# astojanov/Clover

Hardware: AMD Instinct MI355X
Metric: int4 GEMV (CloverMatrix4::mvm) effective GB/s, algorithmic operand bytes / time (higher is better)
Workload: dtype int4; 1 GPU; CloverMatrix4::mvm 65536x65536 int4 (65536x65536 per GPU; preset c3: BASELINE configs[2] per GPU), x and result CloverVector4, STOCHASTIC_ROUNDING_DISABLED, bit-exact reference order; rows_per_gpu=65536, cols=65536, parallelism=row-shard x1, settle_launches=168

## Files before the change

### clover_amd/csrc/matrix4.hip

```cpp
#include "rng_device.h"

#include <stdlib.h>
#include <string.h>


#define MVM_CHUNK 65536u

template <int U, bool NT>
__device__ __forceinline__ void mvm_steps(const u32x4 *__restrict__ Ap, const u32x4 *xs, const float *cs, int q,
                                          uint32_t t0, float &a0, float &a1, float &a2, float &a3)
{
    u32x4 a[U];
#pragma unroll
    for (int u = 0; u < U; u++) a[u] = NT ? __builtin_nontemporal_load(&Ap[4 * (t0 + u) + q]) : Ap[4 * (t0 + u) + q];
#pragma unroll
    for (int u = 0; u < U; u++) {
        const u32x4 xv = xs[4 * (t0 + u) + q];
        const float c = cs[2 * (t0 + u) + (q >> 1)];
        a0 = __builtin_fmaf(c, (float)sdot8(a[u].x, xv.x, 0), a0);
        a1 = __builtin_fmaf(c, (float)sdot8(a[u].y, xv.y, 0), a1);
        a2 = __builtin_fmaf(c, (float)sdot8(a[u].z, xv.z, 0), a2);
        a3 = __builtin_fmaf(c, (float)sdot8(a[u].w, xv.w, 0), a3);
    }
}

template <int U, bool NT>
__device__ __forceinline__ void mvm_steps8(const u32x2 *__restrict__ Ap, const u32x2 *xs, const float *cs, int e, uint32_t t0, float &a0,
                                           float &a1)
{
    u32x2 a[U];
#pragma unroll
    for (int u = 0; u < U; u++) a[u] = NT ? __builtin_nontemporal_load(&Ap[8 * (t0 + u) + e]) : Ap[8 * (t0 + u) + e];
#pragma unroll
    for (int u = 0; u < U; u++) {
        const u32x2 xv = xs[8 * (t0 + u) + e];
        const float c = cs[2 * (t0 + u) + (e >> 2)];
        a0 = __builtin_fmaf(c, (float)sdot8(a[u].x, xv.x, 0), a0);
        a1 = __builtin_fmaf(c, (float)sdot8(a[u].y, xv.y, 0), a1);
    }
}

__device__ __forceinline__ int requantize_wave(float d, float noise, uint32_t *r_words, float *sr, float *scale)
{
    const int lane = threadIdx.x & 63;
    float m = wave_max(__builtin_fabsf(d));
    m = fix_zero_max(m);
    const float k = 7.0f / m;
    const int qv = quant1(d, k, noise);
    if (r_words) {
        uint32_t w = ((uint32_t)qv & 0xFu) << nib_shift(lane & 7);
        w |= __shfl_xor(w, 1);
        w |= __shfl_xor(w, 2);
        w |= __shfl_xor(w, 4);
        if ((lane & 7) == 0) r_words[lane >> 3] = w;
        if (lane == 0) *sr = m;
    }
    *scale = m;
    return qv;
}

struct MvmFuse {
    const uint32_t *qu;
    const float *su;
    float a;
    uint32_t *r2;
    float *sr2;
};

template <int U, bool NT, bool ST, bool FUSE, int L = 4>
__global__ __launch_bounds__(64 * L) void k_m4_mvm64(const uint8_t *__restrict__ A, const float *__restrict__ sA,
                                                  uint64_t cols, const uint8_t *__restrict__ x, const float *__restrict__ sx,
                                                  float *__restrict__ d_out, uint32_t *r, float *sr,
                                                  uint64_t *rng_state, uint64_t seq, const uint64_t *__restrict__ pow_rows, MvmFuse fuse)
{
    extern __shared__ __attribute__((aligned(16))) char smem[];
    u32x4 *xs = reinterpret_cast<u32x4 *>(smem);
    float *cs = reinterpret_cast<float *>(smem + MVM_CHUNK / 2);
    float *dsh = cs + MVM_CHUNK / 64;
    uint64_t *rbase = reinterpret_cast<uint64_t *>(dsh + 64);
    uint64_t *raw = rbase + 4;
    uint64_t *rbase2 = raw + 8, *raw2 = rbase2 + 4;
    if (ST) {
        const uint64_t a0 = rng_workgroup_begin(rng_state, seq, pow_rows, blockIdx.x, 1, (FUSE ? 4ull : 2ull) * gridDim.x, rbase);
        if (FUSE) {
            const uint64_t b2 = wave_pow_apply(pow_rows, a0, (uint64_t)gridDim.x + blockIdx.x, 1);
            if ((threadIdx.x & 63) == 0) rbase2[threadIdx.x >> 6] = b2;
        }
    }
    uint32_t fuse_w = 0;
    float fuse_s = 0.0f;
    if (FUSE && threadIdx.x < 64) {
        fuse_w = fuse.qu[blockIdx.x * 8 + (threadIdx.x >> 3)];
        fuse_s = fuse.su[blockIdx.x];
    }

    static_assert(L == 4 || (L == 8 && !ST), "the stochastic epilogue assumes 4 waves");
    constexpr int THREADS = 64 * L;
    const uint64_t rb = blockIdx.x;
    const int tid = threadIdx.x;
    const int q = tid & (L - 1);
    const int rho = tid / L;
    const uint64_t row = rb * 64 + rho;
    const u32x4 *Arow = reinterpret_cast<const u32x4 *>(A + row * (cols / 2));
    const float *sArow = sA + rb * (cols / 64);

    float a0 = 0.0f, a1 = 0.0f, a2 = 0.0f, a3 = 0.0f;

    for (uint64_t c0 = 0; c0 < cols; c0 += MVM_CHUNK) {
        const uint32_t cw = (uint32_t)((cols - c0) < MVM_CHUNK ? (cols - c0) : MVM_CHUNK);
        if (c0) __syncthreads();
        const u32x4 *xg = reinterpret_cast<const u32x4 *>(x + c0 / 2);
        {
            constexpr int NX = MVM_CHUNK / 32 / THREADS;
            constexpr int NC = MVM_CHUNK / 64 / THREADS;
            u32x4 xr[NX];
            float sa[NC], sv[NC];
            const uint32_t nx = cw / 32, nc = cw / 64;
#pragma unroll
            for (int k = 0; k < NX; k++) { const uint32_t i = tid + THREADS * k; xr[k] = xg[i < nx ? i : 0]; }
#pragma unroll
            for (int k = 0; k < NC; k++) {
                const uint32_t i = tid + THREADS * k, ii = i < nc ? i : 0;
                sa[k] = sArow[c0 / 64 + ii];
                sv[k] = sx[c0 / 64 + ii];
            }
#pragma unroll
            for (int k = 0; k < NX; k++) { const uint32_t i = tid + THREADS * k; if (i < nx) xs[i] = xr[k]; }
#pragma unroll
            for (int k = 0; k < NC; k++) { const uint32_t i = tid + THREADS * k; if (i < nc) cs[i] = (sa[k] * CLV_RCP49) * sv[k]; }
        }
        __syncthreads();

        const u32x4 *Ap = Arow + c0 / 32;
        const uint32_t npairs = cw / 128;
        uint32_t t = 0;
        if constexpr (L == 4) {
            for (; t + U <= npairs; t += U) mvm_steps<U, NT>(Ap, xs, cs, q, t, a0, a1, a2, a3);
            for (; t < npairs; t++) mvm_steps<1, NT>(Ap, xs, cs, q, t, a0, a1, a2, a3);
        } else {
            const u32x2 *Ap8 = reinterpret_cast<const u32x2 *>(Ap);
            const u32x2 *xs8 = reinterpret_cast<const u32x2 *>(xs);
            for (; t + U <= npairs; t += U) mvm_steps8<U, NT>(Ap8, xs8, cs, q, t, a0, a1);
            for (; t < npairs; t++) mvm_steps8<1, NT>(Ap8, xs8, cs, q, t, a0, a1);
        }
    }

    const float v0 = a0 + __shfl_xor(a0, 2);
    const float v1 = a1 + __shfl_xor(a1, 2);
    const float v2 = a2 + __shfl_xor(a2, 2);
    const float v3 = a3 + __shfl_xor(a3, 2);
    const float x0 = v0 + __shfl_xor(v0, 1);
    const float x1 = v1 + __shfl_xor(v1, 1);
    const float x2 = v2 + __shfl_xor(v2, 1);
    const float x3 = v3 + __shfl_xor(v3, 1);
    float dot = (x0 + x2) + (x1 + x3);
    if constexpr (L == 8) {
        const float u0 = a0 + __shfl_xor(a0, 4), u1 = a1 + __shfl_xor(a1, 4);
        const float y0 = u0 + __shfl_xor(u0, 2), y1 = u1 + __shfl_xor(u1, 2);
        const float z0 = y0 + __shfl_xor(y0, 1), z1 = y1 + __shfl_xor(y1, 1);
        dot = z0 + z1;
    }

    if (q == 0) {
        dsh[rho] = dot;
        if (d_out) d_out[row] = dot;
    }
    if (ST && tid < 4) {
        gen_blocks(rbase[tid], 1, raw, tid);
        if (FUSE) gen_blocks(rbase2[tid], 1, raw2, tid);
    }
    __syncthreads();
    if ((r || FUSE) && tid < 64) {
        float noise = 0.0f;
        if (ST) {
            const int grp = tid & 7, j = tid >> 3;
            noise = noise_of(reinterpret_cast<const uint32_t *>(raw + (size_t)(grp >> 2) * 4)[j], grp & 3);
        }
        float m;
        const int qv = requantize_wave(dsh[tid], noise, r ? r + rb * 8 : nullptr, r ? sr + rb : nullptr, &m);
        if (FUSE) {
            const float su7 = div7(fuse_s), sv7 = div7(m * fuse.a);
            const float val = __builtin_fmaf((float)qv, sv7, (float)unpack1(fuse_w, tid & 7) * su7);
            float noise2 = 0.0f;
            if (ST) {
                const int g = (tid & 7) ^ 1, j = tid >> 3;
                noise2 = noise_of(reinterpret_cast<const uint32_t *>(raw2 + (size_t)(g >> 2) * 4)[j], g & 3);
            }
            float m2;
            requantize_wave(val, noise2, fuse.r2 + rb * 8, fuse.sr2 + rb, &m2);
        }
    }
}

__global__ __launch_bounds__(256) void k_m4_quantize_strip(const float *__restrict__ A, uint64_t cols, uint32_t *__restrict__ q,
                                                           float *__restrict__ s, uint32_t strips_x, uint32_t tiles_x)
{
    __shared__ float sh[4][4];
    const uint32_t sj = blockIdx.x % strips_x;
    const uint64_t bi = blockIdx.x / strips_x;
    const int wave = threadIdx.x >> 6, lane = threadIdx.x & 63;
    const uint64_t col = (uint64_t)sj * 256 + 4 * lane;
    const bool live = col < cols;
    const uint64_t row0 = bi * 64 + wave * 16;

    f32x4 v[16];
    float m = 0.0f;
#pragma unroll
    for (int r = 0; r < 16; r++) {
        v[r] = live ? __builtin_nontemporal_load(reinterpret_cast<const f32x4 *>(A + (row0 + r) * cols + col)) : f32x4{0.0f, 0.0f, 0.0f, 0.0f};
        m = fmaxf(m, fmaxf(fmaxf(__builtin_fabsf(v[r].x), __builtin_fabsf(v[r].y)), fmaxf(__builtin_fabsf(v[r].z), __builtin_fabsf(v[r].w))));
    }
    m = row16_max(m);
    if ((lane & 15) == 0) sh[wave][lane >> 4] = m;
    __syncthreads();
    const int t = lane >> 4;
    m = fix_zero_max(fmaxf(fmaxf(sh[0][t], sh[1][t]), fmaxf(sh[2][t], sh[3][t])));
    const float k = 7.0f / m;
    if (wave == 0 && (lane & 15) == 0 && live) s[bi * tiles_x + sj * 4 + t] = m;
    const int odd = lane & 1;
#pragma unroll
    for (int r = 0; r < 16; r += 2) {
        const uint32_t h0 = quant_pack4(v[r], k), h1 = quant_pack4(v[r + 1], k);
        const uint32_t give = odd ? h0 : h1;
        const uint32_t recv = (uint32_t)__builtin_amdgcn_update_dpp(0, (int)give, 0xB1, 0xF, 0xF, false);
        const uint32_t word = odd ? (recv | (h1 << 16)) : (h0 | (recv << 16));
        if (live) __builtin_nontemporal_store(word, &q[((row0 + r + odd) * cols + (col & ~7ull)) / 8]);
    }
}

__global__ __launch_bounds__(256) void k_m4_gemm_simple(const uint8_t *__restrict__ A, const float *__restrict__ sA, uint64_t M,
                                                        uint64_t K, const uint8_t *__restrict__ B, const float *__restrict__ sB,
                                                        uint64_t N, float *__restrict__ C)
{
    const uint64_t j = (uint64_t)blockIdx.x * 16 + (threadIdx.x & 15);
    const uint64_t i = (uint64_t)blockIdx.y * 16 + (threadIdx.x >> 4);
    if (i >= M || j >= N) return;
    const uint64_t kb = K / 64;
    const u32x4 *a = reinterpret_cast<const u32x4 *>(A + i * (K / 2));
    const u32x4 *b = reinterpret_cast<const u32x4 *>(B + j * (K / 2));
    const float *sa = sA + (i >> 6) * kb;
    const float *sb = sB + (j >> 6) * kb;
    float acc = 0.0f;
    for (uint64_t blk = 0; blk < kb; blk++) {
        const int S = dot32(a[2 * blk], b[2 * blk]) + dot32(a[2 * blk + 1], b[2 * blk + 1]);
        const float c = (sa[blk] * CLV_RCP49) * sb[blk];
        acc = __builtin_fmaf(c, (float)S, acc);
    }
    C[i * N + j] = acc;
}

template <bool NT>
__global__ __launch_bounds__(256) void k_m4_restore(const uint32_t *__restrict__ q, const float *__restrict__ s, f32x4 *__restrict__ A,
                                                    uint64_t nquads, uint64_t cols)
{
    const uint64_t f0 = ((uint64_t)blockIdx.x * 4 + (threadIdx.x >> 6)) * 256;
    const int lane = threadIdx.x & 63;
    const uint64_t tiles_x = cols / 64;
    uint32_t wd[4];
    float sc[4];
#pragma unroll
    for (int j = 0; j < 4; j++) {
        const uint64_t f = f0 + 64 * j + lane, fc = f < nquads ? f : 0;
        const uint64_t e = fc * 4, row = e / cols, col = e - row * cols;
        wd[j] = q[fc >> 1];
        sc[j] = s[(row >> 6) * tiles_x + (col >> 6)];
    }
#pragma unroll
    for (int j = 0; j < 4; j++) {
        const uint64_t f = f0 + 64 * j + lane;
        const uint32_t hw = wd[j] >> (16 * (lane & 1));
        const float k = div7(sc[j]);
        f32x4 v;
        v.x = (float)(((int)(hw << 24)) >> 28) * k;
        v.y = (float)(((int)(hw << 28)) >> 28) * k;
        v.z = (float)(((int)(hw << 16)) >> 28) * k;
        v.w = (float)(((int)(hw << 20)) >> 28) * k;
        if (f < nquads) {
            if (NT) __builtin_nontemporal_store(v, &A[f]);
            else A[f] = v;
        }
    }
}

int clm4_quantize_stochastic(const float *A, uint64_t rows, uint64_t cols, int8_t *q, float *s, uint64_t *rng, hipStream_t st);
int clm4_gemm_mfma(const int8_t *A, const float *sA, uint64_t M, uint64_t K, const int8_t *B, const float *sB, uint64_t N, float *C, hipStream_t st);
int clm4_gemm_fp6(const int8_t *A, const float *sA, uint64_t M, uint64_t K, const int8_t *B, const float *sB, uint64_t N, float *C, hipStream_t st);

#define MVM_LDS_BYTES (MVM_CHUNK / 2 + (MVM_CHUNK / 64) * sizeof(float) + 64 * sizeof(float) + 256)

static int launch_mvm(const int8_t *A, const float *sA, uint64_t rows, uint64_t cols, const int8_t *x, const float *sx,
                      float *d, int8_t *r, float *sr, uint64_t *rng, hipStream_t st, const MvmFuse *fuse = nullptr)
{
    const size_t lds = MVM_LDS_BYTES;
    const dim3 grid((unsigned)(rows / 64)), block(256);
    RngTables T = {nullptr, nullptr, nullptr};
    uint64_t seq = 0;
    if (rng) {
        int rc = clv_rng_tables(&T);
        if (rc) return rc;
        seq = clv_rng_seq_for(rng, st);
    }
    const MvmFuse no_fuse = {nullptr, nullptr, 0.0f, nullptr, nullptr};
#define MVM_LAUNCH_F(NT, ST, FUSE)                                                                                               \
    hipLaunchKernelGGL((k_m4_mvm64<8, NT, ST, FUSE>), grid, block, lds, st, (const uint8_t *)A, sA, cols, (const uint8_t *)x, sx, d, \
                       (uint32_t *)r, sr, rng, seq, T.pow_rows, FUSE ? *fuse : no_fuse)
#define MVM_LAUNCH(NT, ST)                                  \
    do {                                                    \
        if (fuse) MVM_LAUNCH_F(NT, ST, true);               \
        else MVM_LAUNCH_F(NT, ST, false);                   \
    } while (0)
    const bool streaming = rows * (cols / 2) > (256ull << 20);
    const bool wide = streaming && !rng && rows / 64 <= 2ull * (uint64_t)clv_cu_count();
    if (wide) {
        if (fuse)
            hipLaunchKernelGGL((k_m4_mvm64<16, true, false, true, 8>), grid, dim3(512), lds, st, (const uint8_t *)A, sA, cols,
                               (const uint8_t *)x, sx, d, (uint32_t *)r, sr, rng, seq, T.pow_rows, *fuse);
        else
            hipLaunchKernelGGL((k_m4_mvm64<16, true, false, false, 8>), grid, dim3(512), lds, st, (const uint8_t *)A, sA, cols,
                               (const uint8_t *)x, sx, d, (uint32_t *)r, sr, rng, seq, T.pow_rows, no_fuse);
    } else if (streaming) {
        if (rng) MVM_LAUNCH(true, true); else MVM_LAUNCH(true, false);
    } else {
        if (rng) MVM_LAUNCH(false, true); else MVM_LAUNCH(false, false);
    }
#undef MVM_LAUNCH
#undef MVM_LAUNCH_F
    CLV_LAUNCH_CHECK();
    return CLV_OK;
}

#ifdef CLV_EXPERIMENTS
__global__ __launch_bounds__(256) void k_read_bw(const u32x4 *__restrict__ p, uint64_t n16, uint32_t *__restrict__ out, int nt)
{
    const uint64_t stride = (uint64_t)gridDim.x * blockDim.x;
    uint32_t acc = 0;
    uint64_t i = (uint64_t)blockIdx.x * blockDim.x + threadIdx.x;
    for (; i + 7 * stride < n16; i += 8 * stride) {
        u32x4 v[8];
#pragma unroll
        for (int u = 0; u < 8; u++) v[u] = nt ? __builtin_nontemporal_load(&p[i + u * stride]) : p[i + u * stride];
#pragma unroll
        for (int u = 0; u < 8; u++) acc ^= v[u].x ^ v[u].y ^ v[u].z ^ v[u].w;
    }
    for (; i < n16; i += stride) { const u32x4 v = p[i]; acc ^= v.x ^ v.y ^ v.z ^ v.w; }
    if (acc == 0x12345678u) out[0] = acc;
}

extern "C" int clvx_read_bw(const void *p, uint64_t bytes, int nt, int blocks_per_cu, void *out, void *stream)
{
    hipLaunchKernelGGL(k_read_bw, dim3(clv_cu_count() * blocks_per_cu), dim3(256), 0, as_stream(stream), (const u32x4 *)p, bytes / 16,
                       (uint32_t *)out, nt);
    CLV_LAUNCH_CHECK();
    return CLV_OK;
}

extern "C" int clvx_mvm_variant(int variant, const int8_t *A, const float *sA, uint64_t rows, uint64_t cols, const int8_t *x,
                                const float *sx, int8_t *r, float *sr, void *stream)
{
    const size_t lds = MVM_LDS_BYTES;
    hipStream_t st = as_stream(stream);
    const dim3 grid((unsigned)(rows / 64)), block(256);
#define CLVX_LAUNCH(U, NT)                                                                                                      \
    hipLaunchKernelGGL((k_m4_mvm64<U, NT, false, false>), grid, block, lds, st, (const uint8_t *)A, sA, cols, (const uint8_t *)x, sx, \
                       (float *)nullptr, (uint32_t *)r, sr, (uint64_t *)nullptr, 0ull, (const uint64_t *)nullptr,                      \
                       MvmFuse{nullptr, nullptr, 0.0f, nullptr, nullptr})
    switch (variant) {
    case 0: CLVX_LAUNCH(8, true); break;
    case 1: CLVX_LAUNCH(8, false); break;
    case 2: CLVX_LAUNCH(4, true); break;
    case 3: CLVX_LAUNCH(16, true); break;
    case 4: CLVX_LAUNCH(2, true); break;
    case 5: CLVX_LAUNCH(16, false); break;
    case 6: CLVX_LAUNCH(32, false); break;
#define CLVX_LAUNCH8(U, NT)                                                                                                       \
    hipLaunchKernelGGL((k_m4_mvm64<U, NT, false, false, 8>), grid, dim3(512), lds, st, (const uint8_t *)A, sA, cols, (const uint8_t *)x, \
                       sx, (float *)nullptr, (uint32_t *)r, sr, (uint64_t *)nullptr, 0ull, (const uint64_t *)nullptr,                 \
                       MvmFuse{nullptr, nullptr, 0.0f, nullptr, nullptr})
    case 7: CLVX_LAUNCH8(8, false); break;
    case 8: CLVX_LAUNCH8(16, false); break;
    case 9: CLVX_LAUNCH8(8, true); break;
    case 10: CLVX_LAUNCH8(16, true); break;
#undef CLVX_LAUNCH8
    default: clv_set_error("clvx_mvm_variant: unknown variant %d", variant); return CLV_ERR_INVALID;
    }
#undef CLVX_LAUNCH
    CLV_LAUNCH_CHECK();
    return CLV_OK;
}
#endif

static int check_mvm_args(const char *fn, const void *A, const void *sA, uint64_t rows, uint64_t cols, const void *x, const void *sx)
{
    CLV_REQUIRE(A && sA && x && sx, "%s: null pointer", fn);
    CLV_REQUIRE(rows % 64 == 0 && cols % 128 == 0, "%s: rows=%llu must be a multiple of 64 and cols=%llu of 128", fn,
                (unsigned long long)rows, (unsigned long long)cols);
    CLV_REQUIRE(rows / 64 <= 0x7FFFFFFFull, "%s: too many rows", fn);
    return CLV_OK;
}

extern "C" int clm4_restore(const int8_t *q, const float *s, uint64_t rows, uint64_t cols, float *A, void *stream)
{
    CLV_REQUIRE(A && q && s, "clm4_restore: null pointer");
    CLV_REQUIRE(rows % 128 == 0 && cols % 128 == 0, "clm4_restore: rows=%llu cols=%llu must be multiples of 128", (unsigned long long)rows,
                (unsigned long long)cols);
    if (!rows || !cols) return CLV_OK;
    const uint64_t nquads = rows * cols / 4, waves = (nquads + 255) / 256;
    CLV_REQUIRE((waves + 3) / 4 <= 0x7FFFFFFFull, "clm4_restore: matrix too large");
    if (rows * cols * sizeof(float) > (256ull << 20))
        hipLaunchKernelGGL(k_m4_restore<true>, dim3((unsigned)((waves + 3) / 4)), dim3(256), 0, as_stream(stream), (const uint32_t *)q, s,
                           (f32x4 *)A, nquads, cols);
    else
        hipLaunchKernelGGL(k_m4_restore<false>, dim3((unsigned)((waves + 3) / 4)), dim3(256), 0, as_stream(stream), (const uint32_t *)q, s,
                           (f32x4 *)A, nquads, cols);
    CLV_LAUNCH_CHECK();
    return CLV_OK;
}

extern "C" int clm4_mvm(const int8_t *A, const float *sA, uint64_t rows, uint64_t cols, const int8_t *x, const float *sx,
                        int8_t *r, float *sr, uint64_t *rng_state_dev, void *stream)
{
    int rc = check_mvm_args("clm4_mvm", A, sA, rows, cols, x, sx);
    if (rc) return rc;
    CLV_REQUIRE(r && sr, "clm4_mvm: null result pointer");
    if (!rows) return CLV_OK;
    hipStream_t st = as_stream(stream);
    return launch_mvm(A, sA, rows, cols, x, sx, nullptr, r, sr, rng_state_dev, st);
}

extern "C" int clm4_mvm_scale_and_add(const int8_t *A, const float *sA, uint64_t rows, uint64_t cols, const int8_t *x, const float *sx,
                                      const int8_t *qu, const float *su, float a, int8_t *t, float *st_, int8_t *r, float *sr,
                                      uint64_t *rng_state_dev, void *stream)
{
    int rc = check_mvm_args("clm4_mvm_scale_and_add", A, sA, rows, cols, x, sx);
    if (rc) return rc;
    CLV_REQUIRE(qu && su && r && sr, "clm4_mvm_scale_and_add: null pointer");
    CLV_REQUIRE((t == nullptr) == (st_ == nullptr), "clm4_mvm_scale_and_add: t and st must both be given or both be NULL");
    CLV_REQUIRE((const void *)r != (const void *)x && (const void *)sr != (const void *)sx,
                "clm4_mvm_scale_and_add: the result must not alias the vector being multiplied");
    if (!rows) return CLV_OK;
    const MvmFuse fuse = {(const uint32_t *)qu, su, a, (uint32_t *)r, sr};
    return launch_mvm(A, sA, rows, cols, x, sx, nullptr, t, st_, rng_state_dev, as_stream(stream), &fuse);
}

extern "C" int clm4_rowdots(const int8_t *A, const float *sA, uint64_t rows, uint64_t cols, const int8_t *x, const float *sx,
                            float *d, void *stream)
{
    int rc = check_mvm_args("clm4_rowdots", A, sA, rows, cols, x, sx);
    if (rc) return rc;
    CLV_REQUIRE(d, "clm4_rowdots: null result pointer");
    if (!rows) return CLV_OK;
    return launch_mvm(A, sA, rows, cols, x, sx, d, nullptr, nullptr, nullptr, as_stream(stream));
}

extern "C" int clm4_quantize(const float *A, uint64_t rows, uint64_t cols, int8_t *q, float *s, uint64_t *rng_state_dev, void *stream)
{
    CLV_REQUIRE(A && q && s, "clm4_quantize: null pointer");
    CLV_REQUIRE(rows % 128 == 0 && cols % 128 == 0, "clm4_quantize: rows=%llu cols=%llu must be multiples of 128",
                (unsigned long long)rows, (unsigned long long)cols);
    if (!rows || !cols) return CLV_OK;
    const uint64_t tiles = (rows / 64) * (cols / 64);
    CLV_REQUIRE(tiles <= 0x7FFFFFFFull, "clm4_quantize: too many tiles");
    if (rng_state_dev) return clm4_quantize_stochastic(A, rows, cols, q, s, rng_state_dev, as_stream(stream));
    const uint32_t strips_x = (uint32_t)((cols + 255) / 256);
    hipLaunchKernelGGL(k_m4_quantize_strip, dim3((unsigned)((rows / 64) * strips_x)), dim3(256), 0, as_stream(stream), A, cols,
                       (uint32_t *)q, s, strips_x, (uint32_t)(cols / 64));
    CLV_LAUNCH_CHECK();
    return CLV_OK;
}

extern "C" int clm4_gemm(const int8_t *A, const float *sA, uint64_t M, uint64_t K, const int8_t *B, const float *sB, uint64_t N,
                         float *C, void *stream)
{
    CLV_REQUIRE(A && sA && B && sB && C, "clm4_gemm: null pointer");
    CLV_REQUIRE(M % 128 == 0 && N % 128 == 0 && K % 128 == 0, "clm4_gemm: M=%llu N=%llu K=%llu must be multiples of 128",
                (unsigned long long)M, (unsigned long long)N, (unsigned long long)K);
    if (!M || !N) return CLV_OK;
    static const int which = [] { const char *e = clv_env("CLV_GEMM_KERNEL"); return !e ? 0 : !strcmp(e, "simple") ? 2 : !strcmp(e, "i8") ? 1 : 0; }();
    if (which == 0 && K > 0) return clm4_gemm_fp6(A, sA, M, K, B, sB, N, C, as_stream(stream));
    if (which == 1 && K > 0) return clm4_gemm_mfma(A, sA, M, K, B, sB, N, C, as_stream(stream));
    hipLaunchKernelGGL(k_m4_gemm_simple, dim3((unsigned)(N / 16), (unsigned)(M / 16)), dim3(256), 0, as_stream(stream),
                       (const uint8_t *)A, sA, M, K, (const uint8_t *)B, sB, N, C);
    CLV_LAUNCH_CHECK();
    return CLV_OK;
}
```

Baseline: 6566 GB/s.

## Overlap x-chunk staging with first A batches and issue A loads before LDS fill

Restructures the chunk loop so the first batch of A row loads is issued before the x vector and scales are staged into LDS. Only the first slice of x is staged up front; the rest is fetched incrementally inside a head loop that also consumes A batches, with a barrier before the remaining steady-state loop. The intent is to hide per-block start-up latency (x staging plus barrier) behind A streaming, at the cost of more complex control flow, explicit waitcnt calls and an extra barrier. It also adds optional timestamp probes and a 32-bit row offset computation.

```diff
diff --git a/clover_amd/csrc/matrix4.hip b/clover_amd/csrc/matrix4.hip
--- a/clover_amd/csrc/matrix4.hip
+++ b/clover_amd/csrc/matrix4.hip
@@ -2,42 +2,45 @@
 
 #include <stdlib.h>
 #include <string.h>
+#include <type_traits>
 
 
 #define MVM_CHUNK 65536u
 
-template <int U, bool NT>
-__device__ __forceinline__ void mvm_steps(const u32x4 *__restrict__ Ap, const u32x4 *xs, const float *cs, int q,
-                                          uint32_t t0, float &a0, float &a1, float &a2, float &a3)
-{
-    u32x4 a[U];
-#pragma unroll
-    for (int u = 0; u < U; u++) a[u] = NT ? __builtin_nontemporal_load(&Ap[4 * (t0 + u) + q]) : Ap[4 * (t0 + u) + q];
+template <int U, bool NT, int L, typename V>
+__device__ __forceinline__ void mvm_load(const V *__restrict__ Ap, int q, uint32_t t0, V (&a)[U])
+{
+    const V *p = Ap + (size_t)L * t0 + q;
+#pragma unroll
+    for (int u = 0; u < U; u++) a[u] = NT ? __builtin_nontemporal_load(&p[L * u]) : p[L * u];
+}
+
+template <int U, int L, typename V>
+__device__ __forceinline__ void mvm_consume(const V (&a)[U], const V *xs, const float *cs, int q, uint32_t t0, float &a0, float &a1,
+                                            float &a2, float &a3)
+{
+    const V *xp = xs + L * t0 + q;
+    const float *cp = cs + 2 * t0 + q / (L / 2);
 #pragma unroll
     for (int u = 0; u < U; u++) {
-        const u32x4 xv = xs[4 * (t0 + u) + q];
-        const float c = cs[2 * (t0 + u) + (q >> 1)];
+        const V xv = xp[L * u];
+        const float c = cp[2 * u];
         a0 = __builtin_fmaf(c, (float)sdot8(a[u].x, xv.x, 0), a0);
         a1 = __builtin_fmaf(c, (float)sdot8(a[u].y, xv.y, 0), a1);
-        a2 = __builtin_fmaf(c, (float)sdot8(a[u].z, xv.z, 0), a2);
-        a3 = __builtin_fmaf(c, (float)sdot8(a[u].w, xv.w, 0), a3);
-    }
-}
-
-template <int U, bool NT>
-__device__ __forceinline__ void mvm_steps8(const u32x2 *__restrict__ Ap, const u32x2 *xs, const float *cs, int e, uint32_t t0, float &a0,
-                                           float &a1)
-{
-    u32x2 a[U];
-#pragma unroll
-    for (int u = 0; u < U; u++) a[u] = NT ? __builtin_nontemporal_load(&Ap[8 * (t0 + u) + e]) : Ap[8 * (t0 + u) + e];
-#pragma unroll
-    for (int u = 0; u < U; u++) {
-        const u32x2 xv = xs[8 * (t0 + u) + e];
-        const float c = cs[2 * (t0 + u) + (e >> 2)];
-        a0 = __builtin_fmaf(c, (float)sdot8(a[u].x, xv.x, 0), a0);
-        a1 = __builtin_fmaf(c, (float)sdot8(a[u].y, xv.y, 0), a1);
-    }
+        if constexpr (L == 4) {
+            a2 = __builtin_fmaf(c, (float)sdot8(a[u].z, xv.z, 0), a2);
+            a3 = __builtin_fmaf(c, (float)sdot8(a[u].w, xv.w, 0), a3);
+        }
+    }
+}
+
+template <int U, bool NT, int L, typename V>
+__device__ __forceinline__ void mvm_steps(const V *__restrict__ Ap, const V *xs, const float *cs, int q, uint32_t t0, float &a0,
+                                          float &a1, float &a2, float &a3)
+{
+    V a[U];
+    mvm_load<U, NT, L>(Ap, q, t0, a);
+    mvm_consume<U, L>(a, xs, cs, q, t0, a0, a1, a2, a3);
 }
 
 __device__ __forceinline__ int requantize_wave(float d, float noise, uint32_t *r_words, float *sr, float *scale)
@@ -71,8 +74,11 @@
 __global__ __launch_bounds__(64 * L) void k_m4_mvm64(const uint8_t *__restrict__ A, const float *__restrict__ sA,
                                                   uint64_t cols, const uint8_t *__restrict__ x, const float *__restrict__ sx,
                                                   float *__restrict__ d_out, uint32_t *r, float *sr,
-                                                  uint64_t *rng_state, uint64_t seq, const uint64_t *__restrict__ pow_rows, MvmFuse fuse)
-{
+                                                  uint64_t *rng_state, uint64_t seq, const uint64_t *__restrict__ pow_rows, MvmFuse fuse
+                                                  CLV_PROBE(, unsigned long long *dbg))
+{
+#define MVM_STAMP(i, when) CLV_PROBE(do { if ((when) && dbg && threadIdx.x == 0) { dbg[blockIdx.x * 8 + (i)] = __builtin_amdgcn_s_memrealtime(); __builtin_amdgcn_s_waitcnt(0xC07F); } } while (0))
+    MVM_STAMP(0, true);
     extern __shared__ __attribute__((aligned(16))) char smem[];
     u32x4 *xs = reinterpret_cast<u32x4 *>(smem);
     float *cs = reinterpret_cast<float *>(smem + MVM_CHUNK / 2);
@@ -89,8 +95,8 @@
     }
     uint32_t fuse_w = 0;
     float fuse_s = 0.0f;
-    if (FUSE && threadIdx.x < 64) {
-        fuse_w = fuse.qu[blockIdx.x * 8 + (threadIdx.x >> 3)];
+    if (FUSE) {
+        fuse_w = fuse.qu[blockIdx.x * 8 + ((threadIdx.x & 63) >> 3)];
         fuse_s = fuse.su[blockIdx.x];
     }
 
@@ -100,50 +106,76 @@
     const int tid = threadIdx.x;
     const int q = tid & (L - 1);
     const int rho = tid / L;
-    const uint64_t row = rb * 64 + rho;
-    const u32x4 *Arow = reinterpret_cast<const u32x4 *>(A + row * (cols / 2));
+    const u32x4 *Arow = reinterpret_cast<const u32x4 *>(A + rb * 64 * (cols / 2) + (uint32_t)rho * (cols / 2));
     const float *sArow = sA + rb * (cols / 64);
 
     float a0 = 0.0f, a1 = 0.0f, a2 = 0.0f, a3 = 0.0f;
 
-    for (uint64_t c0 = 0; c0 < cols; c0 += MVM_CHUNK) {
-        const uint32_t cw = (uint32_t)((cols - c0) < MVM_CHUNK ? (cols - c0) : MVM_CHUNK);
-        if (c0) __syncthreads();
+#define MVM_LOADS_DONE() __builtin_amdgcn_s_waitcnt(0x0F70)
+    constexpr int NX = MVM_CHUNK / 32 / THREADS;
+    constexpr int NC = MVM_CHUNK / 64 / THREADS;
+    constexpr uint32_t HEAD_PAIRS = THREADS / 4;
+    static_assert(HEAD_PAIRS % U == 0 && HEAD_PAIRS >= 2 * U, "a full head is a whole number of batches, at least two");
+    constexpr int HB = HEAD_PAIRS / U, IPB = (NX - 1 + HB - 2) / (HB - 1);
+    using V = typename std::conditional<L == 4, u32x4, u32x2>::type;
+    const V *xsv = reinterpret_cast<const V *>(xs);
+
+    const uint32_t nchunks = (uint32_t)((cols + MVM_CHUNK - 1) / MVM_CHUNK), cw_last = (uint32_t)(cols - (uint64_t)(nchunks - 1) * MVM_CHUNK);
+    for (uint32_t ch = 0; ch < nchunks; ch++) {
+        const uint64_t c0 = (uint64_t)ch * MVM_CHUNK;
+        const uint32_t cw = ch + 1 < nchunks ? MVM_CHUNK : cw_last;
+        const uint32_t nx = cw / 32, nc = cw / 64, npairs = cw / 128;
+        const uint32_t hp = npairs < HEAD_PAIRS ? npairs : HEAD_PAIRS;
+        const V *Ap = reinterpret_cast<const V *>(Arow + c0 / 32);
         const u32x4 *xg = reinterpret_cast<const u32x4 *>(x + c0 / 2);
+        const float *sAc = sArow + c0 / 64, *sxc = sx + c0 / 64;
+
+        V a[U];
+        if (hp >= U) mvm_load<U, NT, L>(Ap, q, 0, a);
         {
-            constexpr int NX = MVM_CHUNK / 32 / THREADS;
-            constexpr int NC = MVM_CHUNK / 64 / THREADS;
-            u32x4 xr[NX];
+            u32x4 xr;
             float sa[NC], sv[NC];
-            const uint32_t nx = cw / 32, nc = cw / 64;
-#pragma unroll
-            for (int k = 0; k < NX; k++) { const uint32_t i = tid + THREADS * k; xr[k] = xg[i < nx ? i : 0]; }
-#pragma unroll
-            for (int k = 0; k < NC; k++) {
-                const uint32_t i = tid + THREADS * k, ii = i < nc ? i : 0;
-                sa[k] = sArow[c0 / 64 + ii];
-                sv[k] = sx[c0 / 64 + ii];
+            if (tid < nx) xr = xg[tid];
+#pragma unroll
+            for (int k = 0; k < NC; k++) { const uint32_t i = tid + THREADS * k; if (i < nc) { sa[k] = sAc[i]; sv[k] = sxc[i]; } }
+            if (ch) __syncthreads();
+            if (tid < nx) xs[tid] = xr;
+#pragma unroll
+            for (int k = 0; k < NC; k++) { const uint32_t i = tid + THREADS * k; if (i < nc) cs[i] = (sa[k] * CLV_RCP49) * sv[k]; }
+        }
+        MVM_LOADS_DONE();
+        __syncthreads();
+        MVM_STAMP(1, ch == 0);
+
+        uint32_t t = 0;
+#pragma clang loop unroll(disable)
+        for (uint32_t b = 0; t + U <= hp; b++, t += U) {
+            const uint32_t bs = __builtin_amdgcn_readfirstlane(b), ts = __builtin_amdgcn_readfirstlane(t);
+            u32x4 xr[IPB];
+#pragma unroll
+            for (int j = 0; j < IPB; j++) {
+                const uint32_t i = tid + THREADS * (1 + (bs - 1) * IPB + j);
+                if (bs && i < nx) xr[j] = xg[i];
             }
-#pragma unroll
-            for (int k = 0; k < NX; k++) { const uint32_t i = tid + THREADS * k; if (i < nx) xs[i] = xr[k]; }
-#pragma unroll
-            for (int k = 0; k < NC; k++) { const uint32_t i = tid + THREADS * k; if (i < nc) cs[i] = (sa[k] * CLV_RCP49) * sv[k]; }
-        }
-        __syncthreads();
-
-        const u32x4 *Ap = Arow + c0 / 32;
-        const uint32_t npairs = cw / 128;
-        uint32_t t = 0;
-        if constexpr (L == 4) {
-            for (; t + U <= npairs; t += U) mvm_steps<U, NT>(Ap, xs, cs, q, t, a0, a1, a2, a3);
-            for (; t < npairs; t++) mvm_steps<1, NT>(Ap, xs, cs, q, t, a0, a1, a2, a3);
-        } else {
-            const u32x2 *Ap8 = reinterpret_cast<const u32x2 *>(Ap);
-            const u32x2 *xs8 = reinterpret_cast<const u32x2 *>(xs);
-            for (; t + U <= npairs; t += U) mvm_steps8<U, NT>(Ap8, xs8, cs, q, t, a0, a1);
-            for (; t < npairs; t++) mvm_steps8<1, NT>(Ap8, xs8, cs, q, t, a0, a1);
-        }
-    }
+            if (bs) mvm_load<U, NT, L>(Ap, q, ts, a);
+            mvm_consume<U, L>(a, xsv, cs, q, ts, a0, a1, a2, a3);
+#pragma unroll
+            for (int j = 0; j < IPB; j++) {
+                const uint32_t i = tid + THREADS * (1 + (bs - 1) * IPB + j);
+                if (bs && i < nx) xs[i] = xr[j];
+            }
+            MVM_LOADS_DONE();
+            MVM_STAMP(2, ch == 0 && b == 0);
+        }
+        if (npairs > hp) {
+            __syncthreads();
+            for (; t + U <= npairs; t += U) mvm_steps<U, NT, L>(Ap, xsv, cs, q, t, a0, a1, a2, a3);
+        }
+        for (; t < npairs; t++) mvm_steps<1, NT, L>(Ap, xsv, cs, q, t, a0, a1, a2, a3);
+        MVM_LOADS_DONE();
+    }
+#undef MVM_LOADS_DONE
+    MVM_STAMP(3, true);
 
     const float v0 = a0 + __shfl_xor(a0, 2);
     const float v1 = a1 + __shfl_xor(a1, 2);
@@ -163,7 +195,7 @@
 
     if (q == 0) {
         dsh[rho] = dot;
-        if (d_out) d_out[row] = dot;
+        if (d_out) d_out[rb * 64 + rho] = dot;
     }
     if (ST && tid < 4) {
         gen_blocks(rbase[tid], 1, raw, tid);
@@ -190,6 +222,8 @@
             requantize_wave(val, noise2, fuse.r2 + rb * 8, fuse.sr2 + rb, &m2);
         }
     }
+    MVM_STAMP(4, true);
+#undef MVM_STAMP
 }
 
 __global__ __launch_bounds__(256) void k_m4_quantize_strip(const float *__restrict__ A, uint64_t cols, uint32_t *__restrict__ q,
@@ -289,7 +323,8 @@
 #define MVM_LDS_BYTES (MVM_CHUNK / 2 + (MVM_CHUNK / 64) * sizeof(float) + 64 * sizeof(float) + 256)
 
 static int launch_mvm(const int8_t *A, const float *sA, uint64_t rows, uint64_t cols, const int8_t *x, const float *sx,
-                      float *d, int8_t *r, float *sr, uint64_t *rng, hipStream_t st, const MvmFuse *fuse = nullptr)
+                      float *d, int8_t *r, float *sr, uint64_t *rng, hipStream_t st, const MvmFuse *fuse = nullptr
+                      CLV_PROBE(, unsigned long long *dbg = nullptr))
 {
     const size_t lds = MVM_LDS_BYTES;
     const dim3 grid((unsigned)(rows / 64)), block(256);
@@ -303,7 +338,7 @@
     const MvmFuse no_fuse = {nullptr, nullptr, 0.0f, nullptr, nullptr};
 #define MVM_LAUNCH_F(NT, ST, FUSE)                                                                                               \
     hipLaunchKernelGGL((k_m4_mvm64<8, NT, ST, FUSE>), grid, block, lds, st, (const uint8_t *)A, sA, cols, (const uint8_t *)x, sx, d, \
-                       (uint32_t *)r, sr, rng, seq, T.pow_rows, FUSE ? *fuse : no_fuse)
+                       (uint32_t *)r, sr, rng, seq, T.pow_rows, FUSE ? *fuse : no_fuse CLV_PROBE(, dbg))
 #define MVM_LAUNCH(NT, ST)                                  \
     do {                                                    \
         if (fuse) MVM_LAUNCH_F(NT, ST, true);               \
@@ -314,10 +349,10 @@
     if (wide) {
         if (fuse)
             hipLaunchKernelGGL((k_m4_mvm64<16, true, false, true, 8>), grid, dim3(512), lds, st, (const uint8_t *)A, sA, cols,
-                               (const uint8_t *)x, sx, d, (uint32_t *)r, sr, rng, seq, T.pow_rows, *fuse);
+                               (const uint8_t *)x, sx, d, (uint32_t *)r, sr, rng, seq, T.pow_rows, *fuse CLV_PROBE(, dbg));
         else
             hipLaunchKernelGGL((k_m4_mvm64<16, true, false, false, 8>), grid, dim3(512), lds, st, (const uint8_t *)A, sA, cols,
-                               (const uint8_t *)x, sx, d, (uint32_t *)r, sr, rng, seq, T.pow_rows, no_fuse);
+                               (const uint8_t *)x, sx, d, (uint32_t *)r, sr, rng, seq, T.pow_rows, no_fuse CLV_PROBE(, dbg));
     } else if (streaming) {
         if (rng) MVM_LAUNCH(true, true); else MVM_LAUNCH(true, false);
     } else {
@@ -363,7 +398,7 @@
 #define CLVX_LAUNCH(U, NT)                                                                                                      \
     hipLaunchKernelGGL((k_m4_mvm64<U, NT, false, false>), grid, block, lds, st, (const uint8_t *)A, sA, cols, (const uint8_t *)x, sx, \
                        (float *)nullptr, (uint32_t *)r, sr, (uint64_t *)nullptr, 0ull, (const uint64_t *)nullptr,                      \
-                       MvmFuse{nullptr, nullptr, 0.0f, nullptr, nullptr})
+                       MvmFuse{nullptr, nullptr, 0.0f, nullptr, nullptr}, (unsigned long long *)nullptr)
     switch (variant) {
     case 0: CLVX_LAUNCH(8, true); break;
     case 1: CLVX_LAUNCH(8, false); break;
@@ -375,7 +410,7 @@
 #define CLVX_LAUNCH8(U, NT)                                                                                                       \
     hipLaunchKernelGGL((k_m4_mvm64<U, NT, false, false, 8>), grid, dim3(512), lds, st, (const uint8_t *)A, sA, cols, (const uint8_t *)x, \
                        sx, (float *)nullptr, (uint32_t *)r, sr, (uint64_t *)nullptr, 0ull, (const uint64_t *)nullptr,                 \
-                       MvmFuse{nullptr, nullptr, 0.0f, nullptr, nullptr})
+                       MvmFuse{nullptr, nullptr, 0.0f, nullptr, nullptr}, (unsigned long long *)nullptr)
     case 7: CLVX_LAUNCH8(8, false); break;
     case 8: CLVX_LAUNCH8(16, false); break;
     case 9: CLVX_LAUNCH8(8, true); break;
@@ -386,6 +421,14 @@
 #undef CLVX_LAUNCH
     CLV_LAUNCH_CHECK();
     return CLV_OK;
+}
+
+extern "C" int clvx_mvm_stamps(const int8_t *A, const float *sA, uint64_t rows, uint64_t cols, const int8_t *x, const float *sx,
+                               int8_t *r, float *sr, unsigned long long *dbg, void *stream)
+{
+    CLV_REQUIRE(A && sA && x && sx && r && sr && dbg, "clvx_mvm_stamps: null pointer");
+    CLV_REQUIRE(rows && rows % 64 == 0 && cols % 128 == 0, "clvx_mvm_stamps: rows must be a multiple of 64 and cols of 128");
+    return launch_mvm(A, sA, rows, cols, x, sx, nullptr, r, sr, nullptr, as_stream(stream), nullptr, dbg);
 }
 #endif
 
```

New measurement: 6328 GB/s. 0.964x the previous value.
